# waiwnf/pilotguru

Hardware: AMD Instinct MI355X
Metric: frames/sec ORB extract+match, 1080p @ 2000 kp/frame (higher is better)
Workload: dtype u8

## Files before the change

pilotguru_amd/csrc/quadtree.hip:

```cpp
#include "pgorb_internal.h"

#define QT_TMAX 1024
#define QT_T ((int)blockDim.x)
#define QT_SH (__builtin_ctz(blockDim.x))
#define QT_W (QT_T >> 6)
#define QT_POS_MASK 0x0FFFFFFFu

#ifndef QT_HU
#define QT_HU 4
#endif
#define QT_SETTLE4(a, b, c, d) asm volatile("" : "+v"(a), "+v"(b), "+v"(c), "+v"(d))

__device__ __forceinline__ int qt_wave_incl_scan(int x)
{
    int v = x;
    v += __builtin_amdgcn_update_dpp(0, v, 0x111, 0xf, 0xf, true);
    v += __builtin_amdgcn_update_dpp(0, v, 0x112, 0xf, 0xf, true);
    v += __builtin_amdgcn_update_dpp(0, v, 0x114, 0xf, 0xf, true);
    v += __builtin_amdgcn_update_dpp(0, v, 0x118, 0xf, 0xf, true);
    v += __builtin_amdgcn_update_dpp(0, v, 0x142, 0xa, 0xf, false);
    v += __builtin_amdgcn_update_dpp(0, v, 0x143, 0xc, 0xf, false);
    return v;
}

__device__ int qt_scan_excl(int* a, int n, int* sh)
{
    const int tid = threadIdx.x, lane = tid & 63, wv = tid >> 6;
    const int per = (n + QT_T - 1) >> QT_SH;
    const int b = tid * per, e = min(b + per, n);
    int sum = 0;
    for (int i = b; i < e; i++) sum += a[i];
    const int incl = qt_wave_incl_scan(sum);
    if (lane == 63) sh[wv] = incl;
    __syncthreads();
    if (wv == 0) {
        const int v = (lane < QT_W) ? sh[lane] : 0;
        const int w = qt_wave_incl_scan(v);
        if (lane < QT_W) sh[lane] = w - v;
        if (lane == QT_W - 1) sh[QT_W] = w;
    }
    __syncthreads();
    int run = sh[wv] + incl - sum;
    for (int i = b; i < e; i++) { const int v = a[i]; a[i] = run; run += v; }
    const int total = sh[QT_W];
    __syncthreads();
    return total;
}

__device__ __forceinline__ void qt_scan3_threads(int& a, int& b, int& c, int* tot, int* sh)
{
    const int tid = threadIdx.x, lane = tid & 63, wv = tid >> 6;
    const int ia = qt_wave_incl_scan(a), ib = qt_wave_incl_scan(b), ic = qt_wave_incl_scan(c);
    if (lane == 63) { sh[wv] = ia; sh[QT_W + wv] = ib; sh[2 * QT_W + wv] = ic; }
    __syncthreads();
    int pa = 0, pb = 0, pc = 0, ta = 0, tb = 0, tc = 0;
    for (int w = 0; w < QT_W; w++) {
        const int va = sh[w], vb = sh[QT_W + w], vc = sh[2 * QT_W + w];
        if (w < wv) { pa += va; pb += vb; pc += vc; }
        ta += va; tb += vb; tc += vc;
    }
    a = pa + ia - a; b = pb + ib - b; c = pc + ic - c;
    tot[0] = ta; tot[1] = tb; tot[2] = tc;
    __syncthreads();
}

__device__ __forceinline__ void qt_wave_count(int* ctr, int target, bool active)
{
    const unsigned long long todo = __ballot(active);
    if (todo == 0) return;
    const int leader = __ffsll((long long)todo) - 1;
    const int t = __builtin_amdgcn_readlane(target, leader);
    if (__ballot(active && target != t) == 0) {
        if ((int)(threadIdx.x & 63) == leader) atomicAdd(&ctr[t], __popcll(todo));
    } else if (active) {
        atomicAdd(&ctr[target], 1);
    }
}

__device__ __forceinline__ int qt_quadrant(const int4 b, uint32_t cv)
{
    const int midX = b.x + ((b.z - b.x + 1) >> 1);
    const int midY = b.y + ((b.w - b.y + 1) >> 1);
    const int x = cv & 0xFFF, y = (cv >> 12) & 0xFFF;
    return (x < midX) ? ((y < midY) ? 0 : 2) : ((y < midY) ? 1 : 3);
}


__device__ __forceinline__ int qt_leaf(uint32_t cv, float hX, int nIni, int regionH, int D)
{
    const int x = cv & 0xFFF, y = (cv >> 12) & 0xFFF;
    int r = (int)__fdiv_rn((float)x, hX);
    r = min(max(r, 0), nIni - 1);
    int x0 = (int)__fmul_rn(hX, (float)r), x1 = (int)__fmul_rn(hX, (float)(r + 1)), y0 = 0, y1 = regionH;
    int idx = r;
    for (int d = 0; d < D; d++) {
        const int midX = x0 + ((x1 - x0 + 1) >> 1), midY = y0 + ((y1 - y0 + 1) >> 1);
        const bool qx = x >= midX, qy = y >= midY;
        idx = idx * 4 + (qx ? 1 : 0) + (qy ? 2 : 0);
        x0 = qx ? midX : x0; x1 = qx ? x1 : midX;
        y0 = qy ? midY : y0; y1 = qy ? y1 : midY;
    }
    return idx;
}

__device__ __forceinline__ int qt_walk(const int* map, int leaf, int nIni, int D)
{
    for (int d = 0; d <= D; d++) {
        const int m = map[qt_pyr_off(nIni, d) + (leaf >> (2 * (D - d)))];
        if (m >= 0) return m;
    }
    return 0;
}

__device__ __forceinline__ int qt_build_keys(const int32_t* __restrict__ cc, const uint32_t* __restrict__ slots, int ncells, int cellCap,
                                             int* cellOff, int* sh, uint2* keys, float hX, int nIni, int regionH, int D)
{
    const int tid = threadIdx.x;
    for (int i = tid; i < ncells; i += QT_T) cellOff[i] = min(cc[i], cellCap);
    __syncthreads();
    const int ncand = qt_scan_excl(cellOff, ncells, sh);
    if (tid == 0) cellOff[ncells] = ncand;
    __syncthreads();
    int steps = 0;
    while ((1 << steps) < ncells) steps++;
    for (int b0 = 0; b0 < ncand; b0 += QT_HU * QT_T) {
        int lo[QT_HU], hi[QT_HU];
#pragma unroll
        for (int u = 0; u < QT_HU; u++) { lo[u] = 0; hi[u] = ncells - 1; }
        for (int st = 0; st < steps; st++) {
#pragma unroll
            for (int u = 0; u < QT_HU; u++) {
                const int mid = (lo[u] + hi[u] + 1) >> 1;
                const bool le = cellOff[mid] <= b0 + u * QT_T + tid;
                lo[u] = le ? mid : lo[u];
                hi[u] = le ? hi[u] : mid - 1;
            }
        }
        uint32_t v[QT_HU];
#pragma unroll
        for (int u = 0; u < QT_HU; u++) {
            const int i = b0 + u * QT_T + tid;
            v[u] = (i < ncand) ? slots[(int64_t)lo[u] * cellCap + (i - cellOff[lo[u]])] : 0u;
        }
        QT_SETTLE4(v[0], v[1], v[2], v[3]);
        if (QT_HU == 8) QT_SETTLE4(v[4 % QT_HU], v[5 % QT_HU], v[6 % QT_HU], v[7 % QT_HU]);
#pragma unroll
        for (int u = 0; u < QT_HU; u++) {
            const int i = b0 + u * QT_T + tid;
            if (i < ncand) keys[i] = make_uint2(v[u], (uint32_t)qt_leaf(v[u], hX, nIni, regionH, D));
        }
    }
    __syncthreads();
    return ncand;
}

template <bool BIG, int WIDE>
__global__ __launch_bounds__((WIDE == 1 || WIDE == 3) ? 512 : QT_TMAX, WIDE == 3 ? 6 : (WIDE ? 4 : 8)) void k_quadtree(const PgPlan P, int level0, int leafOffInts, int split)
{
    __shared__ int sh[3 * (QT_TMAX / 64) + 8];
    __shared__ int pyr[QT_PYR_CAP];
    extern __shared__ __attribute__((aligned(16))) int qt_lds[];
    const int tid = threadIdx.x;
    const int l = level0 + blockIdx.y, frame = blockIdx.x;
    const PgLevel& L = P.lvl[l];
    int* kpc = &P.kpCount[frame * PG_MAXL + l];
    uint2* keys = reinterpret_cast<uint2*>(P.cand) + ((int64_t)frame * P.candFrame + L.candOff);
    if (BIG != (L.nodeOff >= 0)) return;
    const int NC = L.nodeCap;
    int* nodeBase = BIG ? P.nodeScratch + (int64_t)frame * P.nodeFrame + L.nodeOff : qt_lds;
    int4* bndA = reinterpret_cast<int4*>(nodeBase);
    int4* bndB = bndA + NC;
    int* cntA = reinterpret_cast<int*>(bndB + NC);
    int* cntB = cntA + NC;
    int* pidA = cntB + NC;
    int* pidB = pidA + NC;
    int* cnt4 = pidB + NC;
    int* cnt4n = cnt4 + 4 * NC;
    int* newpos4 = cnt4n + 4 * NC;
    int* tailpos = newpos4 + 4 * NC;
    int* rnk = tailpos + NC;
    int* ord = rnk + NC;
    int* cinc = ord + NC;
    int* tmp = newpos4;
    int* ecnt = newpos4 + NC;
    unsigned long long* best = reinterpret_cast<unsigned long long*>(newpos4);
    uint32_t* leafBest = reinterpret_cast<uint32_t*>(qt_lds + leafOffInts);
    int* cellOff = qt_lds + leafOffInts;

    const int N = L.quota;
    const int regionH = L.h - 2 * PG_EDGE;
    const int nIni = L.nIni;
    const float hX = L.hX;
    const int D = qt_pyr_depth(nIni);
    const int pyrTotal = qt_pyr_off(nIni, D + 1);

    const int wCell = L.wCell, hCell = L.hCell, nCols = L.nCols;
    const uint32_t mW = ((1u << 20) + wCell - 1) / wCell, mH = ((1u << 20) + hCell - 1) / hCell;
    auto order_rank = [&](uint32_t cv) {
        const uint32_t x = (cv & 0xFFF) - 3, y = ((cv >> 12) & 0xFFF) - 3;
        const uint32_t cj = (x * mW) >> 20, ci = (y * mH) >> 20;
        return ((ci * nCols + cj) * hCell + (y - ci * hCell)) * wCell + (x - cj * wCell);
    };
    auto bid = [&](uint32_t cv) { return ((unsigned long long)(cv >> 24) << 32) | (0xFFFFFFFFu - order_rank(cv)); };
    const bool rank24 = (long long)L.nCols * L.nRows * hCell * wCell <= (1 << 24);

    int ncand;
    bool keysBuilt = false;
    {
        const int ncells = L.nCols * L.nRows;
        const int32_t* cc = P.cellCount + (int64_t)frame * P.totalCells + L.cellBase;
        const uint32_t* slots = P.cellCand + (int64_t)frame * P.cellCandFrame + L.cellCandOff;
        const int nleaf = nIni << (2 * D);
        for (int i = tid; i < pyrTotal; i += QT_T) pyr[i] = 0;
        if (!split) for (int i = tid; i < nleaf; i += QT_T) leafBest[i] = 0u;
        if (tid == 0) sh[QT_W + 2] = 0;
        int mine = 0;
        const int lane = tid & 63;
        if (split) {
            __syncthreads();
            int* hDs = pyr + qt_pyr_off(nIni, D);
            uint2* gl = P.qtLeaf + ((int64_t)frame * P.nlevels + l) * PG_QT_LEAF_CAP;
            for (int i = tid; i < nleaf; i += QT_T) {
                const uint2 e = gl[i];
                hDs[i] = (int)e.x; leafBest[i] = e.y; mine += (int)e.x;
            }
        } else {
        const int regionW = L.w - 2 * PG_EDGE;
        uint2* xTab = reinterpret_cast<uint2*>(qt_lds);
        uint2* yTab = xTab + regionW;
        for (int i = tid; i < regionW + regionH; i += QT_T) {
            const bool isY = i >= regionW;
            const int c = isY ? i - regionW : i;
            (isY ? yTab : xTab)[c] = qt_tab_entry(isY, c, hX, nIni, regionH, D, wCell, hCell, nCols);
        }
        __syncthreads();
        int* hD = pyr + qt_pyr_off(nIni, D);
        const int wv = __builtin_amdgcn_readfirstlane(tid >> 6);
        const int cellCap = L.cellCap;
        struct __attribute__((packed, aligned(4))) U4 { uint32_t e[4]; };
        if (ncells < QT_T) {
            const int sub = lane >> 4, sl = lane & 15;
            const int cpw = (((ncells + QT_W - 1) >> (QT_SH - 6)) + 31) & ~31;
            const int cBeg = wv * cpw, cEnd = min(ncells, cBeg + cpw);
            int cntNext = (lane < 32 && cBeg + lane < cEnd) ? cc[cBeg + lane] : 0;
            for (int cb = cBeg; cb < cEnd; cb += 32) {
                const int myc = min(cntNext, cellCap);
                cntNext = (lane < 32 && cb + 32 + lane < cEnd) ? cc[cb + 32 + lane] : 0;
                mine += myc;
                int n[8];
                int maxn = myc;
#pragma unroll
                for (int g = 0; g < 8; g++) n[g] = __shfl(myc, 4 * g + sub);
#pragma unroll
                for (int d = 1; d < 32; d <<= 1) maxn = max(maxn, __shfl_xor(maxn, d));
                maxn = __builtin_amdgcn_readfirstlane(maxn);
                const uint32_t* sp = slots + (int64_t)(cb + sub) * cellCap + sl;
                for (int base = 0; base < maxn; base += 16) {
                    uint32_t v[8];
#pragma unroll
                    for (int g = 0; g < 8; g++) v[g] = (base + sl < n[g]) ? sp[(int64_t)(4 * g) * cellCap + base] : 0u;
                    QT_SETTLE4(v[0], v[1], v[2], v[3]); QT_SETTLE4(v[4], v[5], v[6], v[7]);
#pragma unroll
                    for (int g = 0; g < 8; g++) {
                        if (base + sl < n[g]) {
                            const uint2 tx = xTab[v[g] & 0xFFF], ty = yTab[(v[g] >> 12) & 0xFFF];
                            const int lf = (int)(tx.x | ty.x);
                            atomicAdd(&hD[lf], 1);
                            if (rank24) atomicMax(&leafBest[lf], (v[g] & 0xFF000000u) | (0xFFFFFFu - (tx.y + ty.y)));
                        }
                    }
                }
            }
        } else {
        const int cFirst = 64 * wv;
        int cntNext = (cFirst + lane < ncells) ? cc[cFirst + lane] : 0;
        for (int cb = cFirst; cb < ncells; cb += 64 * QT_W) {
            const int myc = min(cntNext, cellCap);
            cntNext = (cb + 64 * QT_W + lane < ncells) ? cc[cb + 64 * QT_W + lane] : 0;
            mine += myc;
            int maxn = myc;
#pragma unroll
            for (int d = 1; d < 64; d <<= 1) maxn = max(maxn, __shfl_xor(maxn, d));
            maxn = __builtin_amdgcn_readfirstlane(maxn);
            const uint32_t* sp = slots + (int64_t)(cb + lane) * cellCap;
            for (int base = 0; base < maxn; base += 32) {
                U4 r[8];
#pragma unroll
                for (int j = 0; j < 8; j++) {
                    r[j] = U4{{0u, 0u, 0u, 0u}};
                    if (base + 4 * j < myc) r[j] = *reinterpret_cast<const U4*>(sp + base + 4 * j);
                }
                const int lim = min(maxn - base, 32);
#pragma unroll
                for (int j = 0; j < 8; j++) {
                    if (4 * j < lim) {
                        uint2 tx[4], ty[4];
#pragma unroll
                        for (int k = 0; k < 4; k++) {
                            const bool ok = base + 4 * j + k < myc;
                            const uint32_t v = ok ? r[j].e[k] : 0u;
                            tx[k] = xTab[v & 0xFFF]; ty[k] = yTab[(v >> 12) & 0xFFF];
                        }
#pragma unroll
                        for (int k = 0; k < 4; k++) {
                            if (base + 4 * j + k < myc) {
                                const int lf = (int)(tx[k].x | ty[k].x);
                                atomicAdd(&hD[lf], 1);
                                if (rank24) atomicMax(&leafBest[lf], (r[j].e[k] & 0xFF000000u) | (0xFFFFFFu - (tx[k].y + ty[k].y)));
                            }
                        }
                    }
                }
            }
        }
        }
        }
#pragma unroll
        for (int d = 32; d >= 1; d >>= 1) mine += __shfl_xor(mine, d);
        if (lane == 0 && mine) atomicAdd(&sh[QT_W + 2], mine);
        __syncthreads();
        ncand = sh[QT_W + 2];
        if (tid == 0) P.candCount[frame * PG_MAXL + l] = ncand;
        if (ncand <= 0 || nIni < 1) {
            PgSelRec* selE = reinterpret_cast<PgSelRec*>(P.sel) + ((int64_t)frame * P.selFrame + L.selOff);
            for (int p = tid; p < L.selCap; p += QT_T) selE[p].posLevel = 0xFFFFFFFFu;
            if (tid == 0) *kpc = 0;
            if (ncand > 0 && tid == 0) atomicExch(P.status, PGORB_E_TOOSMALL);
            return;
        }
        if (!rank24) {
            qt_build_keys(cc, slots, ncells, L.cellCap, cellOff, sh, keys, hX, nIni, regionH, D);
            keysBuilt = true;
        }
        for (int d = D - 1; d >= 0; d--) {
            const int* src = pyr + qt_pyr_off(nIni, d + 1);
            int* dst = pyr + qt_pyr_off(nIni, d);
            const int cnt = nIni << (2 * d);
            for (int j = tid; j < cnt; j += QT_T) dst[j] = src[4 * j] + src[4 * j + 1] + src[4 * j + 2] + src[4 * j + 3];
            __syncthreads();
        }
    }

    int size;
    {
        if (tid == 0) {
            int pos = 0;
            for (int i = 0; i < nIni; i++) {
                if (pyr[i] > 0) {
                    bndA[pos] = make_int4((int)__fmul_rn(hX, (float)i), 0,
                                          (int)__fmul_rn(hX, (float)(i + 1)), regionH);
                    cntA[pos] = pyr[i];
                    pidA[pos] = i;
                    pos++;
                }
            }
            sh[QT_W + 1] = pos;
        }
        __syncthreads();
        size = sh[QT_W + 1];
        if (D >= 1)
            for (int i = tid; i < 4 * size; i += QT_T) cnt4[i] = pyr[nIni + 4 * pidA[i >> 2] + (i & 3)];
        __syncthreads();
    }

    int sorted_mode = 0, gen = 1;
    bool last = false, pyrMode = true;
    while (!last) {
        if (pyrMode && gen > D) {
            if (!keysBuilt) {
                qt_build_keys(P.cellCount + (int64_t)frame * P.totalCells + L.cellBase, P.cellCand + (int64_t)frame * P.cellCandFrame + L.cellCandOff,
                              L.nCols * L.nRows, L.cellCap, cellOff, sh, keys, hX, nIni, regionH, D);
                keysBuilt = true;
            }
            for (int i = tid; i < pyrTotal; i += QT_T) pyr[i] = -1;
            for (int i = tid; i < 4 * size; i += QT_T) cnt4[i] = 0;
            __syncthreads();
            for (int p = tid; p < size; p += QT_T) {
                const int pid = pidA[p];
                pyr[qt_pyr_off(nIni, pid >> 28) + (pid & QT_POS_MASK)] = p;
            }
            __syncthreads();
            for (int i0 = 0; i0 < ncand; i0 += QT_T) {
                const int i = i0 + tid;
                bool act = i < ncand;
                int tgt = 0;
                if (act) {
                    const uint2 k = keys[i];
                    const int pos = qt_walk(pyr, (int)k.y, nIni, D);
                    uint32_t rec = (uint32_t)pos;
                    act = cntA[pos] > 1;
                    if (act) {
                        const int q = qt_quadrant(bndA[pos], k.x);
                        tgt = pos * 4 + q;
                        rec |= (uint32_t)q << 28;
                    }
                    keys[i].y = rec;
                }
                qt_wave_count(cnt4, tgt, act);
            }
            __syncthreads();
            pyrMode = false;
        }
        const int n = size, prevSize = size;
        const bool fill = pyrMode && gen + 1 <= D;
        const int fillOff = qt_pyr_off(nIni, min(gen + 1, D));
        int jstar = 0;
        if (!sorted_mode) {
            const int per = (n + QT_T - 1) >> QT_SH;
            const int pb = tid * per, pe = min(pb + per, n);
            int se = 0, sc = 0, sx = 0;
            for (int p = pb; p < pe; p++)
                if (cntA[p] > 1) {
                    const int c0 = cnt4[4 * p], c1 = cnt4[4 * p + 1], c2 = cnt4[4 * p + 2], c3 = cnt4[4 * p + 3];
                    se++; sc += (c0 > 0) + (c1 > 0) + (c2 > 0) + (c3 > 0); sx += (c0 > 1) + (c1 > 1) + (c2 > 1) + (c3 > 1);
                }
            int tot[3];
            qt_scan3_threads(se, sc, sx, tot, sh);
            const int m = tot[0], Ctot = tot[1], nToExpand = tot[2];
            size = Ctot + (n - m);
            if (size > NC) { if (tid == 0) atomicExch(P.status, PGORB_E_OVERFLOW); size = min(size, NC); last = true; }
            if (size >= N || size == prevSize) last = true;
            else if (size + 3 * nToExpand > N) sorted_mode = 1;
            int re = se, ce = sc;
            for (int p = pb; p < pe; p++) {
                if (cntA[p] > 1) {
                    const int4 b = bndA[p];
                    const int midX = b.x + ((b.z - b.x + 1) >> 1);
                    const int midY = b.y + ((b.w - b.y + 1) >> 1);
                    const int cq[4] = {cnt4[4 * p], cnt4[4 * p + 1], cnt4[4 * p + 2], cnt4[4 * p + 3]};
                    const int c = (cq[0] > 0) + (cq[1] > 0) + (cq[2] > 0) + (cq[3] > 0);
                    const int cidx = (int)(((uint32_t)pidA[p] & (QT_POS_MASK >> 2)) * 4u);
                    int pos = Ctot - (ce + c);
                    if (pos >= 0 && pos + c <= NC) {
#pragma unroll
                        for (int q = 3; q >= 0; q--) {
                            if (cq[q] <= 0) continue;
                            bndB[pos] = make_int4((q & 1) ? midX : b.x, (q & 2) ? midY : b.y,
                                                  (q & 1) ? b.z : midX, (q & 2) ? b.w : midY);
                            cntB[pos] = cq[q];
                            pidB[pos] = (int)(((uint32_t)gen << 28) | (uint32_t)(cidx + q));
                            if (fill && cq[q] > 1) {
                                const int* h = pyr + fillOff + (cidx + q) * 4;
                                cnt4n[4 * pos] = h[0]; cnt4n[4 * pos + 1] = h[1]; cnt4n[4 * pos + 2] = h[2]; cnt4n[4 * pos + 3] = h[3];
                            }
                            newpos4[4 * p + q] = pos++;
                        }
                    }
                    rnk[p] = 0; re++; ce += c;
                } else {
                    const int pos = min(Ctot + (p - re), NC - 1);
                    bndB[pos] = bndA[p]; cntB[pos] = cntA[p]; pidB[pos] = pidA[p];
                    tailpos[p] = pos; rnk[p] = -1;
                }
            }
        } else {
            for (int p = tid; p < n; p += QT_T) rnk[p] = (cntA[p] > 1) ? 1 : 0;
            __syncthreads();
            const int m = qt_scan_excl(rnk, n, sh);
            if (BIG) {
                for (int p = tid; p < n; p += QT_T) {
                    if (cntA[p] > 1) { tmp[rnk[p]] = p; ecnt[rnk[p]] = cntA[p]; }
                    else rnk[p] = -1;
                }
                __syncthreads();
                for (int i = tid; i < m; i += QT_T) {
                    const int ci = ecnt[i];
                    int rank = 0;
                    for (int j = 0; j < m; j++) {
                        const int cj = ecnt[j];
                        rank += (cj > ci) || (cj == ci && j < i);
                    }
                    ord[rank] = tmp[i];
                    rnk[tmp[i]] = rank;
                }
                __syncthreads();
            } else {
                for (int p = tid; p < n; p += QT_T) {
                    if (cntA[p] > 1) { tmp[rnk[p]] = p; ecnt[rnk[p]] = (int)(((uint32_t)min(cntA[p], 0x1FFFFF) << 11) | (uint32_t)(2047 - rnk[p])); }
                    else rnk[p] = -1;
                }
                __syncthreads();
                const int m4 = m & ~3;
                for (int i = tid; i < m; i += QT_T) {
                    const uint32_t ki = (uint32_t)ecnt[i];
                    int rank = 0;
                    for (int j = 0; j < m4; j += 4) {
                        const uint4 k4 = *reinterpret_cast<const uint4*>(ecnt + j);
                        rank += (k4.x > ki) + (k4.y > ki) + (k4.z > ki) + (k4.w > ki);
                    }
                    for (int j = m4; j < m; j++) rank += (uint32_t)ecnt[j] > ki;
                    ord[rank] = tmp[i];
                    rnk[tmp[i]] = rank;
                }
                __syncthreads();
            }
            for (int r = tid; r < m; r += QT_T) {
                const int p = ord[r];
                cinc[r] = (cnt4[4 * p] > 0) + (cnt4[4 * p + 1] > 0) + (cnt4[4 * p + 2] > 0) + (cnt4[4 * p + 3] > 0);
            }
            __syncthreads();
            qt_scan_excl(cinc, m, sh);
            for (int r = tid; r < m; r += QT_T) {
                const int p = ord[r];
                cinc[r] += (cnt4[4 * p] > 0) + (cnt4[4 * p + 1] > 0) + (cnt4[4 * p + 2] > 0) + (cnt4[4 * p + 3] > 0);
            }
            if (tid == 0) sh[QT_W + 1] = m - 1;
            __syncthreads();
            for (int r = tid; r < m; r += QT_T) {
                const bool now = n + cinc[r] - (r + 1) >= N;
                const bool before = (r > 0) && (n + cinc[r - 1] - r >= N);
                if (now && !before) sh[QT_W + 1] = r;
            }
            __syncthreads();
            jstar = sh[QT_W + 1];
            const int Ctot = (m > 0) ? cinc[jstar] : 0;
            for (int p = tid; p < n; p += QT_T) tailpos[p] = (rnk[p] >= 0 && rnk[p] <= jstar) ? 0 : 1;
            __syncthreads();
            const int U = qt_scan_excl(tailpos, n, sh);
            for (int p = tid; p < n; p += QT_T) {
                const int r = rnk[p];
                if (r >= 0 && r <= jstar) {
                    const int4 b = bndA[p];
                    const int midX = b.x + ((b.z - b.x + 1) >> 1);
                    const int midY = b.y + ((b.w - b.y + 1) >> 1);
                    const int cq[4] = {cnt4[4 * p], cnt4[4 * p + 1], cnt4[4 * p + 2], cnt4[4 * p + 3]};
                    const int cidx = (int)(((uint32_t)pidA[p] & (QT_POS_MASK >> 2)) * 4u);
                    int pos = Ctot - cinc[r];
#pragma unroll
                    for (int q = 3; q >= 0; q--) {
                        if (cq[q] <= 0) continue;
                        bndB[pos] = make_int4((q & 1) ? midX : b.x, (q & 2) ? midY : b.y,
                                              (q & 1) ? b.z : midX, (q & 2) ? b.w : midY);
                        cntB[pos] = cq[q];
                        pidB[pos] = (int)(((uint32_t)gen << 28) | (uint32_t)(cidx + q));
                        if (fill && cq[q] > 1) {
                            const int* h = pyr + fillOff + (cidx + q) * 4;
                            cnt4n[4 * pos] = h[0]; cnt4n[4 * pos + 1] = h[1]; cnt4n[4 * pos + 2] = h[2]; cnt4n[4 * pos + 3] = h[3];
                        }
                        newpos4[4 * p + q] = pos++;
                    }
                } else {
                    const int pos = Ctot + tailpos[p];
                    bndB[pos] = bndA[p]; cntB[pos] = cntA[p]; pidB[pos] = pidA[p];
                    tailpos[p] = pos;
                    if (fill && cntA[p] > 1) {
                        cnt4n[4 * pos] = cnt4[4 * p]; cnt4n[4 * pos + 1] = cnt4[4 * p + 1];
                        cnt4n[4 * pos + 2] = cnt4[4 * p + 2]; cnt4n[4 * pos + 3] = cnt4[4 * p + 3];
                    }
                }
            }
            size = Ctot + U;
            if (size > NC) { if (tid == 0) atomicExch(P.status, PGORB_E_OVERFLOW); size = NC; last = true; }
            if (size >= N || size == prevSize) last = true;
        }
        if (!pyrMode) {
            for (int i = tid; i < 4 * size; i += QT_T) cnt4n[i] = 0;
            __syncthreads();
            for (int b0 = 0; b0 < ncand; b0 += 4 * QT_T) {
                uint2 kk[4];
#pragma unroll
                for (int u = 0; u < 4; u++) { const int i = b0 + tid + u * QT_T; kk[u] = (i < ncand) ? keys[i] : make_uint2(0u, 0u); }
        QT_SETTLE4(kk[0].x, kk[1].x, kk[2].x, kk[3].x); QT_SETTLE4(kk[0].y, kk[1].y, kk[2].y, kk[3].y);
                int tgt[4];
                bool act[4];
#pragma unroll
                for (int u = 0; u < 4; u++) {
                    const int i = b0 + tid + u * QT_T;
                    act[u] = i < ncand;
                    tgt[u] = 0;
                    if (act[u]) {
                        const uint2 k = kk[u];
                        const int pos = k.y & QT_POS_MASK, q = k.y >> 28;
                        const int r = rnk[pos];
                        const int np = (r >= 0 && r <= jstar) ? newpos4[4 * pos + q] : tailpos[pos];
                        uint32_t rec = (uint32_t)np;
                        act[u] = !last && cntB[np] > 1;
                        if (act[u]) {
                            const int q2 = qt_quadrant(bndB[np], k.x);
                            tgt[u] = np * 4 + q2;
                            rec |= (uint32_t)q2 << 28;
                        }
                        if (last) atomicMax(&reinterpret_cast<unsigned long long*>(cnt4n)[np], bid(k.x));
                        else keys[i].y = rec;
                    }
                }
#pragma unroll
                for (int u = 0; u < 4; u++) qt_wave_count(cnt4n, tgt[u], act[u]);
            }
        }
        __syncthreads();
        { int4* t4 = bndA; bndA = bndB; bndB = t4; int* t1 = cntA; cntA = cntB; cntB = t1;
          t1 = cnt4; cnt4 = cnt4n; cnt4n = t1; t1 = pidA; pidA = pidB; pidB = t1; }
        gen++;
    }

    if (pyrMode) {
        for (int p = tid; p < size; p += QT_T) best[p] = 0ull;
        int* leafPos = pyr + qt_pyr_off(nIni, D);
        for (int i = tid; i < pyrTotal; i += QT_T) pyr[i] = -1;
        __syncthreads();
        for (int p = tid; p < size; p += QT_T) {
            const int pid = pidA[p];
            pyr[qt_pyr_off(nIni, pid >> 28) + (pid & QT_POS_MASK)] = p;
        }
        __syncthreads();
        const int nleaf = nIni << (2 * D);
        if (!keysBuilt) {
            for (int j = tid; j < nleaf; j += QT_T) {
                const uint32_t k = leafBest[j];
                if (k) atomicMax(&best[qt_walk(pyr, j, nIni, D)], ((unsigned long long)(k >> 24) << 32) | (0xFF000000u | (k & 0xFFFFFFu)));
            }
        } else {
            for (int j = tid; j < nleaf; j += QT_T) leafPos[j] = qt_walk(pyr, j, nIni, D);
            __syncthreads();
            for (int b0 = 0; b0 < ncand; b0 += 4 * QT_T) {
                uint2 kk[4];
#pragma unroll
                for (int u = 0; u < 4; u++) { const int i = b0 + tid + u * QT_T; kk[u] = (i < ncand) ? keys[i] : make_uint2(0u, 0u); }
                QT_SETTLE4(kk[0].x, kk[1].x, kk[2].x, kk[3].x); QT_SETTLE4(kk[0].y, kk[1].y, kk[2].y, kk[3].y);
#pragma unroll
                for (int u = 0; u < 4; u++) {
                    const int i = b0 + tid + u * QT_T;
                    if (i >= ncand) break;
                    atomicMax(&best[leafPos[kk[u].y]], bid(kk[u].x));
                }
            }
        }
    } else {
        best = reinterpret_cast<unsigned long long*>(cnt4);
    }
    __syncthreads();
    PgSelRec* sel = reinterpret_cast<PgSelRec*>(P.sel) + ((int64_t)frame * P.selFrame + L.selOff);
    PgSelRec proto;
    proto.cv = 0; proto.posLevel = (uint32_t)l << 16; proto.pitch = L.pitch; proto.wh = (uint32_t)L.w | ((uint32_t)L.h << 16);
    proto.plane = (uint64_t)(uintptr_t)(L.img + (int64_t)frame * L.fstride); proto.scale = L.scale; proto.patchSize = L.patchSize;
    const int nsel = min(size, L.selCap);
    if (size > L.selCap && tid == 0) atomicExch(P.status, PGORB_E_OVERFLOW);
    const int tileCap = min(1024, 4 * NC - 2);
    int tsh = 6;
    while ((((L.w - 2 * PG_EDGE) >> tsh) + 1) * (((L.h - 2 * PG_EDGE) >> tsh) + 1) > tileCap) tsh++;
    const int tilesX = ((L.w - 2 * PG_EDGE) >> tsh) + 1;
    int* hist = pyrMode ? cnt4 : cnt4n;
    int* wRec = cntA;
    int* wKey = cntB;
    for (int i = tid; i <= tileCap; i += QT_T) hist[i] = 0;
    __syncthreads();
    for (int p = tid; p < nsel; p += QT_T) {
        const unsigned long long b = best[p];
        uint32_t cv = 0u;
        if (b) {
            const uint32_t rank = 0xFFFFFFFFu - (uint32_t)b;
            const uint32_t t1 = rank / (uint32_t)wCell, xr = rank - t1 * (uint32_t)wCell;
            const uint32_t cidx = t1 / (uint32_t)hCell, yr = t1 - cidx * (uint32_t)hCell;
            const uint32_t ci = cidx / (uint32_t)nCols, cj = cidx - ci * (uint32_t)nCols;
            cv = (cj * wCell + xr + 3u) | ((ci * hCell + yr + 3u) << 12) | ((uint32_t)(b >> 32) << 24);
        }
        const int t = (int)(((cv >> 12) & 0xFFF) >> tsh) * tilesX + (int)((cv & 0xFFF) >> tsh);
        wRec[p] = (int)cv;
        wKey[p] = (t << 16) | atomicAdd(&hist[t], 1);
    }
    __syncthreads();
    qt_scan_excl(hist, tileCap + 1, sh);
    for (int p = tid; p < nsel; p += QT_T) {
        const int wk = wKey[p];
        PgSelRec r = proto;
        r.cv = (uint32_t)wRec[p]; r.posLevel |= (uint32_t)p;
        sel[hist[wk >> 16] + (wk & 0xFFFF)] = r;
    }
    for (int p = nsel + tid; p < L.selCap; p += QT_T) sel[p].posLevel = 0xFFFFFFFFu;
    if (tid == 0) *kpc = nsel;
}

#define QTP_T 512
__global__ __launch_bounds__(QTP_T) void k_qt_leaves(const PgPlan P, int level0, int nlev)
{
    extern __shared__ __attribute__((aligned(16))) int qp_lds[];
    const int tid = threadIdx.x, frame = blockIdx.y, lane = tid & 63;
    int rem = blockIdx.x, l = level0;
    for (int k = 0; k < nlev; k++) {
        const PgLevel& V = P.lvl[level0 + k];
        const int g = qt_pass_groups(V.nCols * V.nRows, qt_pyr_depth(V.nIni));
        l = level0 + k;
        if (rem < g) break;
        rem -= g;
    }
    const PgLevel& L = P.lvl[l];
    const int nIni = L.nIni, nCols = L.nCols, ncells = nCols * L.nRows, cellCap = L.cellCap, hCell = L.hCell;
    const int32_t* cc = P.cellCount + (int64_t)frame * P.totalCells + L.cellBase;
    if (nIni < 1) {
        if (rem == 0) {
            int any = 0;
            for (int i = tid; i < ncells; i += QTP_T) any |= cc[i];
            if (any) atomicExch(P.status, PGORB_E_TOOSMALL);
        }
        return;
    }
    const int D = qt_pyr_depth(nIni), rows = 1 << D, ncol = nIni << D;
    const int rowsPer = qt_pass_rows_per_group(ncells, D);
    const int r0 = rem * rowsPer, r1 = min(rows, r0 + rowsPer);
    const int regionW = L.w - 2 * PG_EDGE, regionH = L.h - 2 * PG_EDGE;
    const uint2* gx = P.qtTab + L.qtTabOff;
    const uint2* gy = gx + regionW;
    const uint2* gr = gy + regionH;
    const int ya = (int)gr[r0].x, yb = (int)gr[r1].x;
    uint2* xT = reinterpret_cast<uint2*>(qp_lds);
    uint2* yT = xT + regionW;
    const int nh = (r1 - r0) * ncol;
    int* hC = reinterpret_cast<int*>(yT + (yb - ya));
    uint32_t* hB = reinterpret_cast<uint32_t*>(hC + nh + 64);
    for (int i = tid; i < regionW; i += QTP_T) xT[i] = gx[i];
    for (int i = tid; i < yb - ya; i += QTP_T) { uint2 e = gy[ya + i]; e.x = (e.x - (uint32_t)r0) * (uint32_t)ncol; yT[i] = e; }
    for (int i = tid; i < 2 * (nh + 64); i += QTP_T) hC[i] = 0;
    const uint32_t* slots = P.cellCand + (int64_t)frame * P.cellCandFrame + L.cellCandOff;
    const bool rank24 = (long long)ncells * hCell * L.wCell <= (1 << 24);
    const int ciBeg = max(ya - 3, 0) / hCell, ciEnd = min(L.nRows - 1, max(yb - 1 - 3, 0) / hCell);
    const int c0 = ciBeg * nCols, c1 = (yb > ya) ? (ciEnd + 1) * nCols : c0;
    const int wv = __builtin_amdgcn_readfirstlane(tid >> 6);
    const int cFirst = c0 + 64 * wv;
    int cntNext = (cFirst + lane < c1) ? cc[cFirst + lane] : 0;
    __syncthreads();
    struct __attribute__((packed, aligned(4))) U4 { uint32_t e[4]; };
    for (int cb = cFirst; cb < c1; cb += 64 * (QTP_T / 64)) {
        const int myc = min(cntNext, cellCap);
        cntNext = (cb + 64 * (QTP_T / 64) + lane < c1) ? cc[cb + 64 * (QTP_T / 64) + lane] : 0;
        int maxn = myc;
#pragma unroll
        for (int d = 1; d < 64; d <<= 1) maxn = max(maxn, __shfl_xor(maxn, d));
        maxn = __builtin_amdgcn_readfirstlane(maxn);
        const uint32_t* sp = slots + (int64_t)(cb + lane) * cellCap;
        for (int base = 0; base < maxn; base += 32) {
            U4 r[8];
#pragma unroll
            for (int j = 0; j < 8; j++) {
                r[j] = U4{{0u, 0u, 0u, 0u}};
                if (base + 4 * j < myc) r[j] = *reinterpret_cast<const U4*>(sp + base + 4 * j);
            }
            const int lim = min(maxn - base, 32);
#pragma unroll
            for (int j = 0; j < 8; j++) {
                if (4 * j < lim) {
                    uint2 tx[4], ty[4];
                    bool ok[4];
#pragma unroll
                    for (int k = 0; k < 4; k++) {
                        const uint32_t v = r[j].e[k];
                        const int ys = (int)((v >> 12) & 0xFFF);
                        ok[k] = base + 4 * j + k < myc && ys >= ya && ys < yb;
                        tx[k] = xT[ok[k] ? (v & 0xFFF) : 0u]; ty[k] = yT[ok[k] ? ys - ya : 0];
                    }
#pragma unroll
                    for (int k = 0; k < 4; k++) {
                        const int hi = ok[k] ? (int)(tx[k].x + ty[k].x) : nh + lane;
                        atomicAdd(&hC[hi], 1);
                        if (rank24) atomicMax(&hB[hi], (r[j].e[k] & 0xFF000000u) | (0xFFFFFFu - (tx[k].y + ty[k].y)));
                    }
                }
            }
        }
    }
    __syncthreads();
    uint2* gl = P.qtLeaf + ((int64_t)frame * P.nlevels + l) * PG_QT_LEAF_CAP;
    const uint32_t cmask = (1u << D) - 1;
    for (int i = tid; i < nh; i += QTP_T) {
        const uint32_t rl = (uint32_t)i / (uint32_t)ncol, col = (uint32_t)i - rl * (uint32_t)ncol, row = (uint32_t)r0 + rl;
        const uint32_t leaf = ((col >> D) << (2 * D)) + qt_spread_bits(col & cmask) + 2u * qt_spread_bits(row);
        gl[leaf] = make_uint2((uint32_t)hC[i], hB[i]);
    }
}

void pg_launch_quadtree(const PgPlan& P, int nframes, hipStream_t s) { pg_launch_quadtree_levels(P, nframes, 0, P.nlevels, s); }

void pg_launch_quadtree_levels(const PgPlan& P, int nframes, int levelBeg, int levelEnd, hipStream_t s)
{
    int nodes[2] = {0, 0}, aux[2] = {0, 0};
    bool any[2] = {false, false};
    for (int l = levelBeg; l < levelEnd; l++) {
        const int big = P.lvl[l].nodeOff >= 0 ? 1 : 0;
        const int cells = P.lvl[l].nCols * P.lvl[l].nRows + 1;
        const int nIni = max(P.lvl[l].nIni, 1);
        const int leaves = nIni << (2 * qt_pyr_depth(nIni));
        any[big] = true;
        aux[big] = max(aux[big], max(cells, leaves));
        nodes[big] = max(nodes[big], 2 * ((P.lvl[l].w - 2 * PG_EDGE) + (P.lvl[l].h - 2 * PG_EDGE)));
        if (!big) nodes[0] = max(nodes[0], P.lvl[l].nodeCap * 28);
    }
    static size_t configuredDev[64] = {0};
    int dev = 0;
    (void)hipGetDevice(&dev);
    size_t& configured = configuredDev[dev & 63];
    const int cells0 = P.lvl[levelBeg].nCols * P.lvl[levelBeg].nRows;
    const bool split = P.qtSplit == 1 || (P.qtSplit == 2 && cells0 >= 1500 && nframes <= 16 + (cells0 - 2304) * 12 / 6912);
    if (split) {
        int groups = 0;
        size_t lds = 0;
        for (int l = levelBeg; l < levelEnd; l++) {
            const PgLevel& V = P.lvl[l];
            const int D = qt_pyr_depth(V.nIni), ncells = V.nCols * V.nRows;
            groups += qt_pass_groups(ncells, D);
            lds = std::max(lds, (size_t)((V.w - 2 * PG_EDGE) + (V.h - 2 * PG_EDGE)) * 8 + (size_t)qt_pass_rows_per_group(ncells, D) * (std::max(V.nIni, 0) << D) * 8 + 2 * 64 * 4);
        }
        static size_t passConfigured[64] = {0};
        int dev0 = 0;
        (void)hipGetDevice(&dev0);
        if (lds > 48 * 1024 && lds > passConfigured[dev0 & 63]) {
            (void)hipFuncSetAttribute(reinterpret_cast<const void*>(k_qt_leaves), hipFuncAttributeMaxDynamicSharedMemorySize, (int)lds);
            passConfigured[dev0 & 63] = lds;
        }
        if (groups > 0)
            hipLaunchKernelGGL(k_qt_leaves, dim3(groups, nframes), dim3(QTP_T), lds, s, P, levelBeg, levelEnd - levelBeg);
    }
    for (int big = 0; big < 2; big++) {
        if (!any[big]) continue;
        const size_t lds = (size_t)(nodes[big] + aux[big]) * sizeof(int);
        const size_t ldsAll = lds + sizeof(int) * (QT_PYR_CAP + 3 * (QT_TMAX / 64) + 8);
        int threads = QT_TMAX;
        if (ldsAll <= 80 * 1024 && (cells0 < 1024 || (int64_t)nframes * (levelEnd - levelBeg) > 256)) threads = 512;
        if (P.qtThreads == 256 || P.qtThreads == 512 || P.qtThreads == 1024) threads = P.qtThreads;
        dim3 grid(nframes, levelEnd - levelBeg), block(threads);
        const int64_t problems = (int64_t)nframes * (levelEnd - levelBeg);
        int wide = 0;
        if (P.qtWide && threads == 512 && ldsAll > 54 * 1024) wide = 1;
        if (P.qtWide && threads == 512 && ldsAll > 40 * 1024 && ldsAll <= 54 * 1024) wide = 3;
        if (P.qtWide && threads == QT_TMAX && (ldsAll > 80 * 1024 || problems <= 256)) wide = 2;
        if (lds > configured) {
#define PG_QT_ATTR(B, W) (void)hipFuncSetAttribute(reinterpret_cast<const void*>(k_quadtree<B, W>), hipFuncAttributeMaxDynamicSharedMemorySize, (int)lds)
            PG_QT_ATTR(true, 0); PG_QT_ATTR(true, 1); PG_QT_ATTR(true, 2); PG_QT_ATTR(true, 3); PG_QT_ATTR(false, 0); PG_QT_ATTR(false, 1); PG_QT_ATTR(false, 2); PG_QT_ATTR(false, 3);
#undef PG_QT_ATTR
            configured = lds;
        }
#define PG_QT_LAUNCH(B, W) hipLaunchKernelGGL((k_quadtree<B, W>), grid, block, lds, s, P, levelBeg, nodes[big], split ? 1 : 0)
        if (big) { if (wide == 1) PG_QT_LAUNCH(true, 1); else if (wide == 2) PG_QT_LAUNCH(true, 2); else if (wide == 3) PG_QT_LAUNCH(true, 3); else PG_QT_LAUNCH(true, 0); }
        else { if (wide == 1) PG_QT_LAUNCH(false, 1); else if (wide == 2) PG_QT_LAUNCH(false, 2); else if (wide == 3) PG_QT_LAUNCH(false, 3); else PG_QT_LAUNCH(false, 0); }
#undef PG_QT_LAUNCH
    }
}
```

Before: 100,300.

## Run small pyramid levels and first quadtree generations in a single wavefront

```diff
diff --git a/pilotguru_amd/csrc/quadtree.hip b/pilotguru_amd/csrc/quadtree.hip
--- a/pilotguru_amd/csrc/quadtree.hip
+++ b/pilotguru_amd/csrc/quadtree.hip
@@ -5,6 +5,10 @@
 #define QT_SH (__builtin_ctz(blockDim.x))
 #define QT_W (QT_T >> 6)
 #define QT_POS_MASK 0x0FFFFFFFu
+#define QT_TAIL 256
+#define QT_HS (3 * (QT_TMAX / 64) + 4)
+#define QT_WAVE_SYNC() do { __builtin_amdgcn_fence(__ATOMIC_RELEASE, "wavefront"); __builtin_amdgcn_wave_barrier(); \
+                            __builtin_amdgcn_fence(__ATOMIC_ACQUIRE, "wavefront"); } while (0)
 
 #ifndef QT_HU
 #define QT_HU 4
@@ -204,7 +208,7 @@
     auto bid = [&](uint32_t cv) { return ((unsigned long long)(cv >> 24) << 32) | (0xFFFFFFFFu - order_rank(cv)); };
     const bool rank24 = (long long)L.nCols * L.nRows * hCell * wCell <= (1 << 24);
 
-    int ncand;
+    int ncand, dTail;
     bool keysBuilt = false;
     {
         const int ncells = L.nCols * L.nRows;
@@ -332,39 +336,177 @@
             qt_build_keys(cc, slots, ncells, L.cellCap, cellOff, sh, keys, hX, nIni, regionH, D);
             keysBuilt = true;
         }
-        for (int d = D - 1; d >= 0; d--) {
+        for (dTail = D - 1; dTail >= 0 && (nIni << (2 * dTail)) > QT_TAIL; dTail--) {
+            const int* src = pyr + qt_pyr_off(nIni, dTail + 1);
+            int* dst = pyr + qt_pyr_off(nIni, dTail);
+            const int cnt = nIni << (2 * dTail);
+            for (int j = tid; j < cnt; j += QT_T) dst[j] = src[4 * j] + src[4 * j + 1] + src[4 * j + 2] + src[4 * j + 3];
+            __syncthreads();
+        }
+    }
+
+    if (__builtin_amdgcn_readfirstlane(tid >> 6) == 0) {
+        const int lane = tid;
+        for (int d = dTail; d >= 0; d--) {
             const int* src = pyr + qt_pyr_off(nIni, d + 1);
             int* dst = pyr + qt_pyr_off(nIni, d);
             const int cnt = nIni << (2 * d);
-            for (int j = tid; j < cnt; j += QT_T) dst[j] = src[4 * j] + src[4 * j + 1] + src[4 * j + 2] + src[4 * j + 3];
-            __syncthreads();
-        }
-    }
-
-    int size;
-    {
-        if (tid == 0) {
-            int pos = 0;
-            for (int i = 0; i < nIni; i++) {
-                if (pyr[i] > 0) {
-                    bndA[pos] = make_int4((int)__fmul_rn(hX, (float)i), 0,
-                                          (int)__fmul_rn(hX, (float)(i + 1)), regionH);
-                    cntA[pos] = pyr[i];
-                    pidA[pos] = i;
-                    pos++;
-                }
-            }
-            sh[QT_W + 1] = pos;
-        }
-        __syncthreads();
-        size = sh[QT_W + 1];
-        if (D >= 1)
-            for (int i = tid; i < 4 * size; i += QT_T) cnt4[i] = pyr[nIni + 4 * pidA[i >> 2] + (i & 3)];
-        __syncthreads();
-    }
-
-    int sorted_mode = 0, gen = 1;
-    bool last = false, pyrMode = true;
+            for (int j = lane; j < cnt; j += 64) dst[j] = src[4 * j] + src[4 * j + 1] + src[4 * j + 2] + src[4 * j + 3];
+            QT_WAVE_SYNC();
+        }
+        int n;
+        if (nIni <= 64) {
+            const bool in = lane < nIni;
+            const int i = in ? lane : 0;
+            const int v = pyr[i];
+            int c4[4] = {0, 0, 0, 0};
+            if (D >= 1) { c4[0] = pyr[nIni + 4 * i]; c4[1] = pyr[nIni + 4 * i + 1]; c4[2] = pyr[nIni + 4 * i + 2]; c4[3] = pyr[nIni + 4 * i + 3]; }
+            const unsigned long long has = __ballot(in && v > 0);
+            const int pos = (int)__builtin_amdgcn_mbcnt_hi((uint32_t)(has >> 32), __builtin_amdgcn_mbcnt_lo((uint32_t)has, 0u));
+            if (in && v > 0) {
+                bndA[pos] = make_int4((int)__fmul_rn(hX, (float)i), 0, (int)__fmul_rn(hX, (float)(i + 1)), regionH);
+                cntA[pos] = v;
+                pidA[pos] = i;
+                if (D >= 1) { cnt4[4 * pos] = c4[0]; cnt4[4 * pos + 1] = c4[1]; cnt4[4 * pos + 2] = c4[2]; cnt4[4 * pos + 3] = c4[3]; }
+            }
+            n = __builtin_amdgcn_readfirstlane(__popcll(has));
+        } else {
+            if (lane == 0) {
+                int pos = 0;
+                for (int i = 0; i < nIni; i++) {
+                    if (pyr[i] > 0) {
+                        bndA[pos] = make_int4((int)__fmul_rn(hX, (float)i), 0,
+                                              (int)__fmul_rn(hX, (float)(i + 1)), regionH);
+                        cntA[pos] = pyr[i];
+                        pidA[pos] = i;
+                        pos++;
+                    }
+                }
+                sh[QT_HS] = pos;
+            }
+            QT_WAVE_SYNC();
+            n = __builtin_amdgcn_readfirstlane(sh[QT_HS]);
+            if (D >= 1)
+                for (int i = lane; i < 4 * n; i += 64) cnt4[i] = pyr[nIni + 4 * pidA[i >> 2] + (i & 3)];
+        }
+        QT_WAVE_SYNC();
+        int g = 1, sm = 0, lst = 0;
+        const int gEnd = min(3, D);
+        int more = __builtin_amdgcn_readfirstlane(gEnd >= 1 ? 1 : 0);
+        while (more) {
+            const int par = (g - 1) & 1;
+            const int4* sb = bndA + par * NC; int4* db = bndA + (1 - par) * NC;
+            const int* sc1 = cntA + par * NC; int* dc1 = cntA + (1 - par) * NC;
+            const int* sp = pidA + par * NC; int* dp = pidA + (1 - par) * NC;
+            const int* s4 = cnt4 + par * 4 * NC; int* d4 = cnt4 + (1 - par) * 4 * NC;
+            const bool fill = g + 1 <= D;
+            const int fillOff = qt_pyr_off(nIni, min(g + 1, D));
+            const int per = (n + 63) >> 6;
+            const int pb = lane * per, pe = min(pb + per, n);
+            int se = 0, sc = 0, sx = 0;
+            const bool one = WIDE != 0 && n <= 64;
+            const bool act1 = one && lane < n;
+            const int p1 = act1 ? lane : 0;
+            int cn1 = 0, pid1 = 0, cq1[4] = {0, 0, 0, 0};
+            int4 b1 = make_int4(0, 0, 0, 0);
+            bool e1 = false;
+            if (one) {
+                cn1 = sc1[p1]; pid1 = sp[p1]; b1 = sb[p1];
+                const int c0 = s4[4 * p1], c1 = s4[4 * p1 + 1], c2 = s4[4 * p1 + 2], c3 = s4[4 * p1 + 3];
+                e1 = act1 && cn1 > 1;
+                cq1[0] = e1 ? c0 : 0; cq1[1] = e1 ? c1 : 0; cq1[2] = e1 ? c2 : 0; cq1[3] = e1 ? c3 : 0;
+                se = e1 ? 1 : 0;
+                sc = (cq1[0] > 0) + (cq1[1] > 0) + (cq1[2] > 0) + (cq1[3] > 0); sx = (cq1[0] > 1) + (cq1[1] > 1) + (cq1[2] > 1) + (cq1[3] > 1);
+            } else
+            for (int p = pb; p < pe; p++)
+                if (sc1[p] > 1) {
+                    const int c0 = s4[4 * p], c1 = s4[4 * p + 1], c2 = s4[4 * p + 2], c3 = s4[4 * p + 3];
+                    se++; sc += (c0 > 0) + (c1 > 0) + (c2 > 0) + (c3 > 0); sx += (c0 > 1) + (c1 > 1) + (c2 > 1) + (c3 > 1);
+                }
+            const int ie = qt_wave_incl_scan(se), ic = qt_wave_incl_scan(sc), ix = qt_wave_incl_scan(sx);
+            const int m = __builtin_amdgcn_readlane(ie, 63), Ctot = __builtin_amdgcn_readlane(ic, 63), nToExpand = __builtin_amdgcn_readlane(ix, 63);
+            int sz = Ctot + (n - m);
+            if (sz > NC) { if (lane == 0) atomicExch(P.status, PGORB_E_OVERFLOW); sz = NC; lst = 1; }
+            if (sz >= N || sz == n) lst = 1;
+            else if (sz + 3 * nToExpand > N) sm = 1;
+            sz = __builtin_amdgcn_readfirstlane(sz); lst = __builtin_amdgcn_readfirstlane(lst); sm = __builtin_amdgcn_readfirstlane(sm);
+            int re = ie - se, ce = ic - sc;
+            if (one) {
+                const int cidx = e1 ? (int)(((uint32_t)pid1 & (QT_POS_MASK >> 2)) * 4u) : 0;
+                int h[4][4];
+                if (fill) {
+#pragma unroll
+                    for (int q = 0; q < 4; q++)
+#pragma unroll
+                        for (int j = 0; j < 4; j++) h[q][j] = pyr[fillOff + (cidx + q) * 4 + j];
+                }
+                if (e1) {
+                    const int midX = b1.x + ((b1.z - b1.x + 1) >> 1);
+                    const int midY = b1.y + ((b1.w - b1.y + 1) >> 1);
+                    int pos = Ctot - ic;
+                    if (pos >= 0 && pos + sc <= NC) {
+#pragma unroll
+                        for (int q = 3; q >= 0; q--) {
+                            if (cq1[q] <= 0) continue;
+                            db[pos] = make_int4((q & 1) ? midX : b1.x, (q & 2) ? midY : b1.y,
+                                                (q & 1) ? b1.z : midX, (q & 2) ? b1.w : midY);
+                            dc1[pos] = cq1[q];
+                            dp[pos] = (int)(((uint32_t)g << 28) | (uint32_t)(cidx + q));
+                            if (fill && cq1[q] > 1) { d4[4 * pos] = h[q][0]; d4[4 * pos + 1] = h[q][1]; d4[4 * pos + 2] = h[q][2]; d4[4 * pos + 3] = h[q][3]; }
+                            pos++;
+                        }
+                    }
+                } else if (act1) {
+                    const int pos = min(Ctot + (p1 - ie), NC - 1);
+                    db[pos] = b1; dc1[pos] = cn1; dp[pos] = pid1;
+                }
+            } else
+            for (int p = pb; p < pe; p++) {
+                if (sc1[p] > 1) {
+                    const int4 b = sb[p];
+                    const int midX = b.x + ((b.z - b.x + 1) >> 1);
+                    const int midY = b.y + ((b.w - b.y + 1) >> 1);
+                    const int cq[4] = {s4[4 * p], s4[4 * p + 1], s4[4 * p + 2], s4[4 * p + 3]};
+                    const int c = (cq[0] > 0) + (cq[1] > 0) + (cq[2] > 0) + (cq[3] > 0);
+                    const int cidx = (int)(((uint32_t)sp[p] & (QT_POS_MASK >> 2)) * 4u);
+                    int pos = Ctot - (ce + c);
+                    if (pos >= 0 && pos + c <= NC) {
+#pragma unroll
+                        for (int q = 3; q >= 0; q--) {
+                            if (cq[q] <= 0) continue;
+                            db[pos] = make_int4((q & 1) ? midX : b.x, (q & 2) ? midY : b.y,
+                                                (q & 1) ? b.z : midX, (q & 2) ? b.w : midY);
+                            dc1[pos] = cq[q];
+                            dp[pos] = (int)(((uint32_t)g << 28) | (uint32_t)(cidx + q));
+                            if (fill && cq[q] > 1) {
+                                const int* h = pyr + fillOff + (cidx + q) * 4;
+                                d4[4 * pos] = h[0]; d4[4 * pos + 1] = h[1]; d4[4 * pos + 2] = h[2]; d4[4 * pos + 3] = h[3];
+                            }
+                            pos++;
+                        }
+                    }
+                    re++; ce += c;
+                } else {
+                    const int pos = min(Ctot + (p - re), NC - 1);
+                    db[pos] = sb[p]; dc1[pos] = sc1[p]; dp[pos] = sp[p];
+                }
+            }
+            QT_WAVE_SYNC();
+            n = sz; g++;
+            more = __builtin_amdgcn_readfirstlane((g <= gEnd && !lst && !sm) ? 1 : 0);
+        }
+        if (lane == 0) { sh[QT_HS] = n; sh[QT_HS + 1] = g; sh[QT_HS + 2] = sm | (lst << 1); }
+    }
+    __syncthreads();
+
+    int size = __builtin_amdgcn_readfirstlane(sh[QT_HS]);
+    int gen = __builtin_amdgcn_readfirstlane(sh[QT_HS + 1]);
+    int sorted_mode = __builtin_amdgcn_readfirstlane(sh[QT_HS + 2]) & 1;
+    bool last = (__builtin_amdgcn_readfirstlane(sh[QT_HS + 2]) >> 1) != 0, pyrMode = true;
+    if (!(gen & 1)) {
+        int4* t4 = bndA; bndA = bndB; bndB = t4; int* t1 = cntA; cntA = cntB; cntB = t1;
+        t1 = cnt4; cnt4 = cnt4n; cnt4n = t1; t1 = pidA; pidA = pidB; pidB = t1;
+    }
     while (!last) {
         if (pyrMode && gen > D) {
             if (!keysBuilt) {
```

After: 100,600 (median of 3 runs). No clear change (+0.3%).
